# yhlleo/DWC-GAN

Hardware: AMD Instinct MI355X
Metric: CelebA 128x128 training images/sec (higher is better)
Workload: dtype f32; 1 GPU; BASELINE configs[1]: CelebA-shaped 128x128, per-GPU batch 16, fp32, full iteration (dis_update + gen_update + EMA + LR step), vgg_w=0, stride-1 3x3 / 5x5 and stride-2 4x4 layers (forward, data and weight gradient) as fp32-accurate TWO-plane f16 split products on the f16 MFMA (hi + lo 2^-11 per operand, per-tensor power-of-two scales, 3 products per multiply-add, matrix-core partial sums flushed to; image_size=128, per_gpu_batch=16, global_batch=16, parallelism=dp1

## Files before the change

### dwc-gan_amd/csrc/conv_halo_x3.hip

```cpp
#include <type_traits>

#include "conv_geom.h"

namespace {

typedef __bf16 bf16;
typedef __bf16 bf16x8 __attribute__((ext_vector_type(8)));
typedef unsigned int u32x2 __attribute__((ext_vector_type(2)));

constexpr int TB = 16;
constexpr int CS = 16;

typedef float f32x2 __attribute__((ext_vector_type(2)));
__device__ __forceinline__ void split3(f32x4 v, u32x2& p0, u32x2& p1, u32x2& p2) {
#pragma unroll
    for (int k = 0; k < 2; ++k) {
        const f32x2 x = {v[2 * k], v[2 * k + 1]};
        const f32x2 hb = {__uint_as_float(__float_as_uint(x[0]) & 0xffff0000u), __uint_as_float(__float_as_uint(x[1]) & 0xffff0000u)};
        const f32x2 r = x - hb;
        const f32x2 mb = {__uint_as_float(__float_as_uint(r[0]) & 0xffff0000u), __uint_as_float(__float_as_uint(r[1]) & 0xffff0000u)};
        const f32x2 l = r - mb;
        p0[k] = __builtin_amdgcn_perm(__float_as_uint(x[1]), __float_as_uint(x[0]), 0x07060302u);
        p1[k] = __builtin_amdgcn_perm(__float_as_uint(r[1]), __float_as_uint(r[0]), 0x07060302u);
        p2[k] = __builtin_amdgcn_perm(__float_as_uint(l[1]), __float_as_uint(l[0]), 0x07060302u);
// ... 32 lines not shown
    const bf16* w;
    const float* bias;
    const float* add;
    float* y;
    int B, H, W, Cin, N, rows, act, reflect;
    int blocks_x, blocks_per_img, tiles_n;
    float* part = nullptr;
    unsigned* tickets = nullptr;
    unsigned* status = nullptr;
    int split_from = 0;
    const unsigned long long* xs = nullptr;
    unsigned xs_epoch = 0;
    size_t w_elems = 0;
    unsigned long long* ys = nullptr;
    unsigned ys_epoch = 0;
};

template <int KS, int BN, int WM, int WN, int TM, int TN, int DBG = 0, int PB = 2, int S2 = 0, int KSP = 1, int NPL = 3, int RING = 0,
          bool ZP = false>
__global__ __launch_bounds__(64 * WM * WN, WM * WN == 4 ? 2 : 1) void conv_halo_x3_kernel(X3Args a) {
    static_assert(!ZP || S2 == 1, "ZP is the stride-2 forward's zero rule (the other forms take X3Args::reflect)");
#if defined(__HIP_DEVICE_COMPILE__)
    constexpr int NW = WM * WN, THREADS = 64 * NW;
    constexpr int PPT = THREADS / 4;
    static_assert((NW == 8 || NW == 4) && WM * TM * 32 == 256 && WN * TN * 32 == BN, "tile shape");
    static_assert(!S2 || KS == 2, "stride-2 form: 2x2 taps per parity");
    static_assert(KSP == 1 || (KSP == 2 && S2 != 2 && NW == 4 && TM * TN <= 4), "contraction split: the two-per-CU tile only");
    static_assert(!RING || (NPL == 2 && PB == 1 && ((S2 == 0 && (KS == 3 || KS == 5)) || S2 == 2)), "fused border ring: two-plane data gradients");
    constexpr int PW = TB + KS - 1;
    constexpr int NALT = RING ? (S2 == 2 ? 1 : ((KS - 1) / 2) * ((KS - 1) / 2 + 1) / 2) : 0;
    constexpr int PWA = PW + NALT;
    constexpr int PPIX = PW * PW;
    constexpr int PPASS = (PPIX + PPT - 1) / PPT;
    constexpr int PITCH = PWA * CS + 8;
    constexpr int P_PLANE = PWA * PITCH;
    constexpr int W_CHUNKS = NPL * BN * 2;
// ... 574 lines not shown
                    }
                    if constexpr (NPL == 2) v = v * sx.inv * sw.inv;
                    v += bv[n][q4];
#pragma unroll
                    for (int k = 0; k < 4; ++k) {
                        if constexpr (decltype(general)::value) v[k] = dwc_act_apply(v[k], a.act, col + k);
                        else v[k] = dwc_act_simple(v[k], slope);
                    }
                    if (a.add) v += adv[n][q4];
                    if constexpr (NPL == 2) y_am = max(max(y_am, max(dwc_abs_bits(v[0]), dwc_abs_bits(v[1]))), max(dwc_abs_bits(v[2]), dwc_abs_bits(v[3])));
                    if (!(DBG & 256)) *reinterpret_cast<f32x4*>(dst + col) = v;
                    else asm volatile("" ::"v"(v));
                }
        }
    };
    if (dwc_act_is_simple(a.act)) store(std::false_type{});
    else store(std::true_type{});
    if constexpr (NPL == 2) {
        __shared__ unsigned s_am[NW];
        dwc_amax_block_publish(a.ys, a.ys_epoch, y_am, s_am);
    }
#endif
}

__global__ void x3_weight_prepare_kernel(const float* __restrict__ w, bf16* __restrict__ out, int Cout, int Cin, int K, int rows,
                                         int kdim, int dgrad) {
    const int ncs = (kdim + CS - 1) / CS;
    const size_t total = (size_t)K * K * ncs * rows * CS;
    const size_t idx = (size_t)blockIdx.x * blockDim.x + threadIdx.x;
    if (idx >= total) return;
    const int j = idx % CS;
    size_t r = idx / CS;
// ... 38 lines not shown
    const int cs = r % ncs, tap = r / ncs;
    const int kh = tap / K, kw = tap - kh * K;
    const int kc = cs * CS + j;
    float v = 0.f;
    if (!dgrad) {
        if (row < Cout && kc < Cin) v = w[(((size_t)row * Cin + kc) * K + kh) * K + kw];
    } else {
        if (row < Cin && kc < Cout) v = w[(((size_t)kc * Cin + row) * K + (K - 1 - kh)) * K + (K - 1 - kw)];
    }
    v *= sw.s;
    const _Float16 h = (_Float16)v;
    const _Float16 l = (_Float16)(v - (float)h);
    const size_t base = ((size_t)(tap * ncs + cs) * 2 * rows + row) * CS + (j ^ (((row >> 3) & 1) << 3));
    out[base] = __builtin_bit_cast(unsigned short, h);
    out[base + (size_t)rows * CS] = __builtin_bit_cast(unsigned short, l);
}

__global__ __launch_bounds__(256) void absmax_kernel(const float* __restrict__ x, size_t n, unsigned long long* slot, unsigned epoch) {
    const size_t n4 = n >> 2;
    unsigned m = 0;
    const f32x4* x4 = reinterpret_cast<const f32x4*>(x);
    const size_t stride = (size_t)gridDim.x * 256;
    size_t i = (size_t)blockIdx.x * 256 + threadIdx.x;
    for (; i + 3 * stride < n4; i += 4 * stride) {
        const f32x4 a = x4[i], b = x4[i + stride], c = x4[i + 2 * stride], d = x4[i + 3 * stride];
#pragma unroll
        for (int k = 0; k < 4; ++k) m = max(max(m, dwc_abs_bits(a[k])), max(dwc_abs_bits(b[k]), max(dwc_abs_bits(c[k]), dwc_abs_bits(d[k]))));
    }
    for (; i < n4; i += stride) {
        const f32x4 a = x4[i];
// ... 312 lines not shown
    for (int c = 1; c <= smax && c * roles <= 2 * cus; ++c) {
        const int wgs = c * roles, rounds = (wgs + cus - 1) / cus;
        const double fill = (double)wgs / (rounds * cus) / (rounds > 1 ? 1.05 : 1.0);
        if (fill > best + 1e-9) best = fill, s = c;
    }
    *ups = (units + s - 1) / s;
    *splits = (units + *ups - 1) / *ups;
}

bool x3_ok(int B, int H, int W, int Cin, int N, int K) {
    return B > 0 && (K == 3 || K == 5) && H >= TB && W >= TB && !(H % TB) && !(W % TB) && Cin >= CS && !(Cin % CS) && N >= 32 &&
           !(N % 4);
}

template <int KS, int BN, int WM, int WN, int TM, int TN, int DBG = 0, int PB = 2, int S2 = 0, int KSP = 1, int NPL = 3, int RING = 0,
          bool ZP = false>
void x3_launch(const X3Args& a, dim3 grid, hipStream_t st) {
    hipLaunchKernelGGL((conv_halo_x3_kernel<KS, BN, WM, WN, TM, TN, DBG, PB, S2, KSP, NPL, RING, ZP>), grid, dim3(64 * WM * WN), 0, st, a);
}
size_t h2_w_elems(int rows, int kdim, int K) { return (size_t)K * K * ((kdim + CS - 1) / CS) * 2 * rows * CS; }

constexpr int X3_KSPLIT_TILES = 256, X3_KSPLIT_TICKETS = 512;
constexpr size_t X3_KSPLIT_TILE_BYTES = 256 * 64 * sizeof(float);
long x3_ksplit_from(long tiles, int slabs) {
    static const int on = getenv("DWC_X3_KSPLIT") ? atoi(getenv("DWC_X3_KSPLIT")) : 1;
    if (!on || slabs < 8 || (slabs & 1) || (tiles & 7)) return -1;
    return tiles <= X3_KSPLIT_TILES ? 0 : -1;
}
bool x3_ksplit_on(long tiles, int slabs) { return x3_ksplit_from(tiles, slabs) >= 0; }
size_t x3_ksplit_bytes(long tiles, int slabs) {
    const long from = x3_ksplit_from(tiles, slabs);
    return from < 0 ? 0 : (size_t)(tiles - from) * X3_KSPLIT_TILE_BYTES;
}
// ... 268 lines not shown

int dwc_x3_conv2d_s2_bwd_data(const float* dy, const void* w_prepared, float* dx, int B, int H, int W, int Cin, int Cout, int rows,
                              void* stream) {
    return x3_s2_bwd_data_impl<3>(dy, nullptr, 0, w_prepared, dx, B, H, W, Cin, Cout, rows, stream);
}
int dwc_h2_conv2d_s2_bwd_data(const float* dy, const void* dy_amax, unsigned dy_epoch, const void* w_prepared, float* dx, int B, int H, int W,
                              int Cin, int Cout, int rows, void* stream) {
    return x3_s2_bwd_data_impl<2>(dy, dy_amax, dy_epoch, w_prepared, dx, B, H, W, Cin, Cout, rows, stream);
}

int dwc_h2_conv2d_s2_bwd_data_fused(const float* dy, const void* dy_amax, unsigned dy_epoch, const void* w_prepared, float* dx, int B, int H,
                                    int W, int Cin, int Cout, int rows, void* stream) {
    return x3_s2_bwd_data_impl<2>(dy, dy_amax, dy_epoch, w_prepared, dx, B, H, W, Cin, Cout, rows, stream, true);
}

size_t dwc_x3_conv2d_wgrad_ws_bytes(int B, int H, int W, int Cin, int Cout, int K) {
    const int bn = x3_wgrad_bn(B, H, W, Cin, Cout, K);
    if (!bn) return 0;
    int splits = 0;
    for (int npl = 2; npl <= 3; ++npl) {
        int s, ups;
        x3_wgrad_plan(B, H, W, Cin, Cout, K, bn, npl, &s, &ups);
        splits = s > splits ? s : splits;
    }
    return (size_t)splits * (bn == 128 ? 1 : 2) * K * K * Cin * Cout * sizeof(float);
}

}

template <int NPL, bool ZP = false>
// ... 63 lines not shown
```

### dwc-gan_amd/hipdwc/_lib.py

```python
import ctypes
import os

_HERE = os.path.dirname(os.path.abspath(__file__))
LIB_PATH = os.environ.get("DWC_HIP_LIB") or os.path.join(os.path.dirname(_HERE), "lib", "libdwcgan_hip.so")

c_fp = ctypes.c_void_p
c_int = ctypes.c_int
c_sz = ctypes.c_size_t
c_f = ctypes.c_float
c_u = ctypes.c_uint


class AdvSpec(ctypes.Structure):
    _fields_ = [("target", c_f * 4), ("w_src", c_f * 4), ("w_cls", c_f * 4)]


BN_MAX_SEGMENTS = 8


TXT_MAX_LAYERS = 4


class TxtLayers(ctypes.Structure):
    _fields_ = [("n", c_int), ("out", c_fp * TXT_MAX_LAYERS), ("c", c_fp * TXT_MAX_LAYERS)]
# ... 129 lines not shown
    "dwc_x3_conv2d_wgrad_ws_bytes": (c_sz, [c_int] * 6),
    "dwc_x3_conv2d_wgrad": (c_int, [c_fp, c_fp, c_fp] + [c_int] * 8 + [c_fp, c_sz, c_fp]),
    "dwc_absmax": (c_int, [c_fp, c_sz, c_fp, c_u, c_fp]),
    "dwc_instnorm_fwd_amax": (c_int, [c_fp] * 7 + [c_int, c_int, c_int, c_f, c_int, c_fp, c_sz, c_fp, c_u, c_fp]),
    "dwc_instnorm_bwd_amax": (c_int, [c_fp] * 9 + [c_int, c_int, c_int, c_int, c_fp, c_sz, c_fp, c_u, c_fp]),
    "dwc_layernorm_fwd_amax": (c_int, [c_fp] * 6 + [c_int, c_int, c_int, c_f, c_int, c_fp, c_sz, c_fp, c_u, c_fp]),
    "dwc_layernorm_bwd_amax": (c_int, [c_fp] * 9 + [c_int, c_int, c_int, c_f, c_int, c_fp, c_sz, c_fp, c_u, c_fp]),
    "dwc_act_bwd_bias_amax": (c_int, [c_fp, c_fp, c_fp, c_fp, c_int, c_int, c_int, c_fp, c_sz, c_fp, c_u, c_fp]),
    "dwc_h2_weight_prepared_elems": (c_sz, [c_int] * 3),
    "dwc_h2_weight_prepare": (c_int, [c_fp, c_fp] + [c_int] * 5 + [c_fp, c_u, c_fp]),
    "dwc_h2_conv2d_same_add_ws": (c_int, [c_fp, c_fp, c_u] + [c_fp] * 4 + [c_fp, c_u] + [c_int] * 9 + [c_fp, c_sz, c_fp, c_fp]),
    "dwc_h2_conv2d_bwd_data_same_fused": (c_int, [c_fp, c_fp, c_u] + [c_fp] * 3 + [c_int] * 7 + [c_fp, c_sz, c_fp, c_fp]),
    "dwc_h2_conv2d_s2_ws": (c_int, [c_fp, c_fp, c_u] + [c_fp] * 3 + [c_fp, c_u] + [c_int] * 7 + [c_fp, c_sz, c_fp, c_fp]),
    "dwc_h2_conv2d_s2_bwd_data": (c_int, [c_fp, c_fp, c_u, c_fp, c_fp] + [c_int] * 6 + [c_fp]),
    "dwc_h2_conv2d_s2_bwd_data_fused": (c_int, [c_fp, c_fp, c_u, c_fp, c_fp] + [c_int] * 6 + [c_fp]),
    "dwc_h2_conv2d_wgrad": (c_int, [c_fp, c_fp, c_u, c_fp, c_fp, c_u, c_fp] + [c_int] * 8 + [c_fp, c_sz, c_fp]),
    "dwc_bf16_conv2d_wgrad_halo_ws_bytes": (c_sz, [c_int] * 6),
    "dwc_bf16_conv2d_wgrad_halo": (c_int, [c_fp, c_fp, c_fp] + [c_int] * 8 + [c_fp, c_sz, c_fp]),
    "dwc_bf16_conv7_smallk_wgrad_ws_bytes": (c_sz, [c_int] * 4),
    "dwc_bf16_conv7_smallk_wgrad": (c_int, [c_fp, c_fp, c_fp] + [c_int] * 5 + [c_fp, c_sz, c_fp]),
    "dwc_x3_conv7_smallk_wgrad_ws_bytes": (c_sz, [c_int] * 4),
    "dwc_x3_conv7_smallk_wgrad": (c_int, [c_fp, c_fp, c_fp] + [c_int] * 5 + [c_fp, c_sz, c_fp]),
    "dwc_bf16_conv2d_stem_ok": (c_int, [c_int] * 7),
    "dwc_bf16_conv2d_stem": (c_int, [c_fp] * 4 + [c_int] * 9 + [c_fp]),
    "dwc_bf16_conv2d_stem_crop": (c_int, [c_fp] * 5 + [c_int] * 10 + [c_fp]),
    "dwc_bf16_conv2d_narrow_ok": (c_int, [c_int] * 8),
    "dwc_bf16_conv2d_narrow": (c_int, [c_fp] * 4 + [c_int] * 12 + [c_fp]),
    "dwc_bf16_conv2d_bwd_data_image_narrow": (c_int, [c_fp, c_fp, c_fp] + [c_int] * 7 + [c_fp, c_sz, c_fp]),
    "dwc_bf16_conv2d_bwd_data_image_ws_bytes": (c_sz, [c_int] * 7),
    "dwc_bf16_conv2d_bwd_data_image": (c_int, [c_fp, c_fp, c_fp] + [c_int] * 7 + [c_fp, c_sz, c_fp]),
# ... 135 lines not shown
```

### dwc-gan_amd/hipdwc/ops.py

```python
import os
import weakref

import numpy as np
import torch

from . import _lib, derived

ACT = {"none": 0, None: 0, "relu": 1, "lrelu": 2, "tanh": 3, "sigmoid": 4, "heads": 5, "heads8": 6}

PRECISION = "fp32"
BF16 = torch.bfloat16

_REMOVED_SWITCHES = ("DWC_WINOGRAD", "DWC_TXT_STREAM", "DWC_NORM_FUSED_FINAL", "DWC_GEMM_TILE", "DWC_STRIP_BM", "DWC_X3_DUO", "DWC_X3_BN",
                     "DWC_X3_BN32", "DWC_X3_WIDE", "DWC_X3_STAGGER", "DWC_HALO_STAGGER", "DWC_X3_WDUO", "DWC_HALO16", "DWC_HALO_DUO",
                     "DWC_HALO_BN128", "DWC_BF16_TILE", "DWC_BF16_STAGES3", "DWC_NARROW_ROWS16")
_set = [k for k in _REMOVED_SWITCHES if k in os.environ]
if _set:
    import warnings
    warnings.warn("hipdwc: %s no longer select%s anything (removed in round 5, DESIGN.md 10.3) and %s ignored" % (
        ", ".join(_set), "s" if len(_set) == 1 else "", "is" if len(_set) == 1 else "are"), stacklevel=2)
del _set


def set_precision(name):
# ... 545 lines not shown

class ResGradToken:
    __slots__ = ("g",)

    def __init__(self):
        self.g = None


RES_FUSE = int(os.environ.get("DWC_RES_FUSE", "1"))


def res_token(x):
    return ResGradToken() if RES_FUSE and torch.is_grad_enabled() and x.requires_grad else None


_X3_TICKETS = {}


def _x3_ksplit(lib, dev, B, H, W, Cx, cop, K, stride, at_least=0):
    need = lib.dwc_x3_conv2d_ksplit_ws_bytes(B, H, W, Cx, cop, K, stride)
    if not need:
        ws = workspace(at_least, dev) if at_least else None
        return ws, at_least, None
    key = (_dev_index(dev), _stream())
    row = _X3_TICKETS.get(key)
    if row is None:
        row = torch.zeros(int(lib.dwc_x3_conv2d_ksplit_ticket_words()), dtype=torch.int32, device=dev)
        _X3_TICKETS[key] = row
    n = max(int(need), int(at_least))
    return workspace(n, dev), n, row.data_ptr()
# ... 148 lines not shown
    if x.dtype == BF16:
        ws = workspace(lib.dwc_bf16_conv7_smallk_wgrad_ws_bytes(B, H, W, int(swapped)), x.device)
        _lib.check(_timed("conv_wgrad_kernel+reduce", flops, lambda: lib.dwc_bf16_conv7_smallk_wgrad(
            a.data_ptr(), bt.data_ptr(), dw.data_ptr(), B, H, W, planes, int(swapped), ws.data_ptr(), ws.numel(), st),
            scope_name=scope_name, detail=kind + shape), "conv7_smallk_wgrad")
    else:
        ws = workspace(lib.dwc_x3_conv7_smallk_wgrad_ws_bytes(B, H, W, int(swapped)), x.device)
        _lib.check(_timed("wgrad_x3_kernel+reduce", flops, lambda: lib.dwc_x3_conv7_smallk_wgrad(
            a.data_ptr(), bt.data_ptr(), dw.data_ptr(), B, H, W, planes, int(swapped), ws.data_ptr(), ws.numel(), st),
            scope_name=scope_name, detail=kind + "-x3" + shape, exec_flops=6 * flops), "x3_conv7_smallk_wgrad")


class _Conv2d(torch.autograd.Function):

    @staticmethod
    def forward(ctx, x, w, b, stride, pad, act, bias_grad=True, owner=None, token=None, nograd=False, zero=False):
        _require_device(x)
        lib = _lib.load()
        x = cl(x)
        half = x.dtype == BF16
        ctx.token = token
        B, Cx, H, W = x.shape
        Cout, Cin, KH, KW = w.shape
        if Cin > Cx:
            raise ValueError("input has %d channels, weight expects %d" % (Cx, Cin))
        ctx.bias_grad = bias_grad
        ctx.zero_flag = bool(b is not None and getattr(b, "_dwc_zero_grad", False))
        ctx.owner = owner
        zero = bool(zero and pad > 0)
        ctx.zero = zero
        refl = 0 if zero else 1
        z = "_zeropad" if zero else ""
        cop = _padc(Cout, x.dtype)
# ... 47 lines not shown
                x.data_ptr(), w_hwio.data_ptr(), _p(bias), y.data_ptr(), B, H, W, Cx, cop, act, st),
                detail="fwd-s2halo" + shape), "conv2d_s2_halo")
        elif half and HALO and stride == 1 and KH == KW and 2 * pad == KH - 1 and lib.dwc_bf16_conv2d_same_halo_ok(B, H, W, Cx, cop, KH):
            _halo_same_bf16(lib, x, w, owner, "fwd", bias, None, y, B, H, W, Cx, cop, KH, act, refl, flops, "fwd-halo" + shape)
        else:
            w_hwio = _prepped(w, "fwd", cop, Cx, stride, owner, half)
            nws = _fn(lib, "conv2d_fwd_ws_bytes", x)(B, H, W, Cx, cop, KH, KW, stride, pad)
            wsp = _splitk_ws(nws, x.device)
            _lib.check(_timed("conv_gemm_kernel", flops, lambda: _fn(lib, "conv2d_fwd_zeropad" if zero else "conv2d_fwd", x)(
                x.data_ptr(), w_hwio.data_ptr(), _p(bias), y.data_ptr(), B, H, W, Cx, cop, KH, KW, stride, pad, act, wsp, nws,
                st), detail="fwd" + shape), "conv2d_fwd")
        ctx.save_for_backward(x, w, y if act != 0 else None)
        ctx.x_amax = getattr(x, "_dwc_amax", None)
        ctx.geom = (B, H, W, Cx, cop, KH, KW, stride, pad, act, Cin, Cout, b is not None)
        ctx.bscope = ("bwd:" + SCOPE) if SCOPE else ""
        return y

    @staticmethod
    def backward(ctx, dy):
        lib = _lib.load()
        x, w, y = ctx.saved_tensors
        B, H, W, Cx, cop, KH, KW, stride, pad, act, Cin, Cout, has_b = ctx.geom
        dy = cl(dy)
        Ho, Wo = dy.shape[2], dy.shape[3]
        need_db = has_b and ctx.needs_input_grad[2]
        g = dy
        db = None
        if need_db and not ctx.bias_grad:
            db, need_db = (None if ctx.zero_flag else torch.zeros(Cout, dtype=torch.float32, device=x.device)), False
        if act != 0 or need_db:
            g, db_full = _act_bwd(lib, dy, y, B, cop, Ho, Wo, act, need_db, slot=True)
            _hbm("act_bwd_bias", dy.numel() * dy.element_size() * ((1 if y is None else 2) + (1 if act != 0 else 0)))
            if need_db:
                db = db_full[:Cout]
        g_res = None
        if ctx.token is not None:
            g_res, ctx.token.g = ctx.token.g, None
            if g_res is not None:
                g_res = cl(g_res)
                if g_res.shape[1] != Cx or g_res.dtype != x.dtype or not ctx.needs_input_grad[0]:
                    raise RuntimeError("residual-gradient token: shape / dtype of the identity branch does not match the block input")
        flops = 2.0 * B * Ho * Wo * Cout * Cin * KH * KW
        shape = " B%d %dx%d %d>%d k%d s%d" % (B, H, W, Cx, cop, KH, stride)
        dx = dw = None
        if ctx.needs_input_grad[1]:
            dw = _Conv2d._wgrad(ctx, lib, x, g, w, flops, shape)
        if ctx.needs_input_grad[0]:
            same = stride == 1 and pad > 0 and 2 * pad == KH - 1 and KH == KW and cop >= 32 and (cop & (cop - 1)) == 0
            dx, used = (_Conv2d._dgrad_zero if ctx.zero else _Conv2d._dgrad_reflect)(ctx, lib, g, g_res, w, same, flops, shape)
            if used:
                g_res = None
        if g_res is not None and dx is not None:
            dx = dx + g_res.to(dx.dtype)
        return dx, dw, db, None, None, None, None, None, None, None, None

    @staticmethod
    def _wgrad(ctx, lib, x, g, w, flops, shape):
        B, H, W, Cx, cop, KH, KW, stride, pad, act, Cin, Cout, has_b = ctx.geom
        half = x.dtype == BF16
        dev, st = x.device, _stream()
        zero = ctx.zero
        dw = torch.empty((Cout, Cin, KH, KW), dtype=torch.float32, device=dev)
        z = "_zeropad" if zero else ""
        if (not zero) and Cout == 64 and (_stem_bf16(half, Cx, cop, KH, KW, stride, pad)
                                          or (SMALLK_X3 and _stem_x3(half, Cx, cop, KH, KW, stride, pad))):
            _smallk_wgrad(lib, x, g, dw, B, H, W, Cin, False, flops, ctx.bscope, "wgrad-stem", shape)
        elif ((not half) and (_x3_use(lib, B, H, W, Cx, cop, KH, KW, stride, pad)
                              or (X3 and X3_S2 and stride == 2 and KH == 4 and KW == 4 and pad == 1))
              and (KH != 3 or X3_WGRAD_HALO3) and (not zero or B * H * W * Cx * 4 < (1 << 31))
# ... 86 lines not shown
                _lib.check(_timed("conv_gemm_kernel", flops, lambda: _fn(lib, "conv2d_bwd_data_same", g)(
                    g.data_ptr(), w_dg(), w_dg_t(), dx.data_ptr(), B, H, W, Cx, cop, KH, KW, pad, ws.data_ptr(),
                    ws.numel(), st), scope_name=ctx.bscope, detail="dgrad" + shape), "conv2d_bwd_data_same")
                return dx, False
            _lib.check(_timed("conv_gemm_kernel" if half else "conv_halo_x3_kernel", 0.0, lambda: _fn(lib, "conv2d_bwd_data_ring", g)(
                g.data_ptr(), w_dg(), w_dg_t(), dx.data_ptr(), B, H, W, Cx, cop, KH, KW, pad, ws.data_ptr(), nws, st),
                scope_name=ctx.bscope, detail="dgrad-ring" + shape), "conv2d_bwd_data_ring")
            return dx, True
        if _s2_dgrad_halo_ok(lib, half, B, H, W, Cx, cop, KH, KW, stride, pad):
            fused = bool(RING_FUSED and (half or h2_fits(g)))
            w_dg = _prepped(w, "dgrad", cop, Cx, 2, owner, half) if half or not fused else None
            if half and fused:
                _lib.check(_timed("conv_gemm_kernel", flops, lambda: lib.dwc_bf16_conv2d_s2_halo_bwd_data_fused(
                    g.data_ptr(), w_dg.data_ptr(), dx.data_ptr(), B, H, W, Cx, cop, st), scope_name=ctx.bscope,
                    detail="dgrad-s2halo" + shape), "conv2d_s2_halo_bwd_data_fused")
            elif fused:
                w_h2 = _prepped(w, "h2_dgrad", cop, Cx, 1, owner)
                ga = amax_of(g)
                _lib.check(_timed("conv_halo_x3_kernel", flops, lambda: lib.dwc_h2_conv2d_s2_bwd_data_fused(
                    g.data_ptr(), ga[0], ga[1], w_h2.data_ptr(), dx.data_ptr(), B, H, W, Cx, cop, Cx, st), scope_name=ctx.bscope,
                    exec_flops=3 * flops, detail="dgrad-h2s2" + shape), "h2_conv2d_s2_bwd_data_fused")
            else:
                dxp = workspace(B * (H + 2) * (W + 2) * Cx * (2 if half else 4), dev)
                _s2_dgrad_halo(lib, g, w, owner, dx, B, H, W, Cx, cop, flops, ctx.bscope, shape)
                _lib.check(_timed("conv_gemm_kernel" if half else "conv_halo_x3_kernel", 0.0, lambda: _fn(lib, "conv2d_bwd_data_s2_ring", g)(
                    g.data_ptr(), w_dg.data_ptr(), dxp.data_ptr(), dx.data_ptr(), B, H, W, Cx, cop, st), scope_name=ctx.bscope,
                    detail="dgrad-ring" + shape), "conv2d_bwd_data_s2_ring")
            return dx, False
        _im2col_dgrad_reflect(lib, g, w, owner, dx, B, H, W, Cx, cop, KH, KW, stride, pad, flops, ctx.bscope, "dgrad" + shape)
        return dx, False

    @staticmethod
# ... 1 lines not shown
        B, H, W, Cx, cop, KH, KW, stride, pad, act, Cin, Cout, has_b = ctx.geom
        owner = ctx.owner
        dt = g.dtype
        half = dt == BF16
        dev = g.device
        dx = empty_cl(B, Cx, H, W, dev, dt)
        if same and (not half) and _x3_use(lib, B, H, W, cop, Cx, KH, KW, stride, pad, free=True):
            _sp_same(lib, g, w, owner, "dgrad", None, g_res, dx, B, H, W, Cx, cop, KH, 0, 0, flops, shape + " zeropad", " zeropad dgrad",
                     scope_name=ctx.bscope)
            return dx, True
        if same and half and HALO and lib.dwc_bf16_conv2d_same_halo_ok(B, H, W, cop, Cx, KH):
            _halo_same_bf16(lib, g, w, owner, "dgrad", None, g_res, dx, B, H, W, Cx, cop, KH, 0, 0, flops, "dgrad-halo" + shape + " zeropad",
                            " zeropad dgrad", ctx.bscope)
            return dx, True
        if _s2_dgrad_halo_ok(lib, half, B, H, W, Cx, cop, KH, KW, stride, pad):
            _s2_dgrad_halo(lib, g, w, owner, dx, B, H, W, Cx, cop, flops, ctx.bscope, shape + " zeropad", " zeropad")
            return dx, False
        w_dg = _prepped(w, "dgrad", cop, Cx, stride, owner, half)
        nws = _fn(lib, "conv2d_bwd_data_crop_ws_bytes", g)(B, H, W, Cx, cop, KH, KW, stride, pad)
        wsp = _splitk_ws(nws, dev)
        st = _stream()
        _lib.check(_timed("conv_gemm_kernel", flops, lambda: _fn(lib, "conv2d_bwd_data_crop", g)(
            g.data_ptr(), w_dg.data_ptr(), dx.data_ptr(), B, H, W, Cx, cop, KH, KW, stride, pad, wsp, nws, st),
            scope_name=ctx.bscope, detail="dgrad" + shape + " zeropad"), "conv2d_bwd_data_crop")
        return dx, False


_PAD_MODES = ("reflect", "zero")


def _pad_mode_zero(pad_mode):
    if pad_mode not in _PAD_MODES:
        raise ValueError("pad_mode %r: the HIP convolutions take %s" % (pad_mode, " / ".join(_PAD_MODES)))
    return pad_mode == "zero"


def conv2d(x, w, b, stride, pad, act="none", bias_grad=True, owner=None, token=None, pad_mode="reflect"):
    zero = _pad_mode_zero(pad_mode)
    if not bias_grad and ZERO_GRAD_BY_FLAG and isinstance(b, torch.nn.Parameter):
        b._dwc_zero_grad = True
    y = _Conv2d.apply(x, w, b, int(stride), int(pad), ACT[act], bool(bias_grad), owner, token, not torch.is_grad_enabled(), zero)
    return y if y.shape[1] == w.shape[0] else y[:, :w.shape[0]]


def conv2d_padded(x, w, b, stride, pad, act="none", pad_mode="reflect"):
    return _Conv2d.apply(x, w, b, int(stride), int(pad), ACT[act], True, None, None, False, _pad_mode_zero(pad_mode))


class _HeadsConvWide(torch.autograd.Function):

    @staticmethod
    def forward(ctx, x, w4, b4, owner=None):
        _require_device(x)
        lib = _lib.load()
        x = cl(x)
        half = x.dtype == BF16
# ... 900 lines not shown
```

### dwc-gan_amd/networks/networks.py

```python
import torch
import torch.nn.functional as F
from torch import nn

from hipdwc import batchnorm, ops, spectral

_CONV_ACTS = ("relu", "lrelu", "tanh", "sigmoid", "none")
_NORM_ACTS = ("relu", "lrelu", "none")


class AdaptiveInstanceNorm2d(nn.Module):

    def __init__(self, num_features, eps=1e-5, momentum=0.1):
        super().__init__()
        self.num_features, self.eps, self.momentum = num_features, eps, momentum
        self.weight = None
        self.bias = None
        self.register_buffer("running_mean", torch.zeros(num_features))
        self.register_buffer("running_var", torch.ones(num_features))

    def forward(self, x, relu=False, residual=None, token=None, act=None):
        if self.weight is None or self.bias is None:
            raise AssertionError("Please assign weight and bias before calling AdaIN!")
        return ops.instance_norm(x, self.weight, self.bias, residual=residual, relu=relu, eps=self.eps, token=token, act=act)

# ... 90 lines not shown
        else:
            raise AssertionError("Unsupported normalization: {}".format(norm))
        if activation == "prelu":
            self.activation = nn.PReLU()
        self.conv = nn.Conv2d(input_dim, output_dim, kernel_size, stride, bias=self.use_bias)
        if norm == "sn":
            self.conv = SpectralNorm(self.conv)

    def _torch_act(self, y):
        if self.act_kind == "prelu":
            return self.activation(y)
        if self.act_kind == "selu":
            return torch.nn.functional.selu(y)
        return {"lrelu": lambda t: torch.nn.functional.leaky_relu(t, 0.1), "tanh": torch.tanh, "sigmoid": torch.sigmoid}[self.act_kind](y)

    def forward(self, x, residual=None, conv_token=None, res_token=None, sn=None, segments=None, stat_order=None):
        if x.shape[1] < 4:
            x = ops.pack_image(x)
        pad = self.padding
        mode = "zero" if self.pad_type == "zero" and ops.ZERO_PAD_HIP else "reflect"
        if self.pad_type != "reflect" and mode != "zero" and pad > 0:
            if self.stride != 1:
                raise NotImplementedError("pad_type=%r with stride %d needs hipdwc.ops.ZERO_PAD_HIP = 1" % (self.pad_type, self.stride))
            x = torch.nn.functional.pad(x, (pad,) * 4, mode="constant" if self.pad_type == "zero" else "replicate")
            pad = 0
        fused_act = self.act_kind in _CONV_ACTS
        if self.norm_kind == "sn":
            if sn is None:
                sn = spectral.sn_power_iteration([self.conv.module], segments or 1)
            y = spectral.sn_conv2d(x, self.conv.module, sn, self.stride, pad, self.act_kind if fused_act else "none", token=conv_token,
                                   pad_mode=mode)
            if not fused_act:
                y = self._torch_act(y)
            return y if residual is None else y + residual
        if self.norm is None:
            y = ops.conv2d(x, self.conv.weight, self.conv.bias, self.stride, pad, self.act_kind if fused_act else "none", token=conv_token,
                           pad_mode=mode)
            if not fused_act:
                y = self._torch_act(y)
            return y if residual is None else y + residual
        if self.norm_kind == "bn":
            bias = self.conv.bias
            train = self.norm.training or not self.norm.track_running_stats
            if not train and getattr(bias, "_dwc_zero_grad", False):
                bias._dwc_zero_grad = False
            y = ops.conv2d(x, self.conv.weight, bias, self.stride, pad, "none", bias_grad=not train, token=conv_token, pad_mode=mode)
            fused = self.act_kind in batchnorm.ACTS
            y = self.norm(y, act=self.act_kind if fused else "none", segments=segments, stat_order=stat_order)
            if not fused:
                y = self._torch_act(y)
            return y if residual is None else y + residual
        if self.act_kind not in (_NORM_ACTS if ops.NORM_ACT_FUSED else ("relu", "none")):
            y = ops.conv2d(x, self.conv.weight, self.conv.bias, self.stride, pad, "none", token=conv_token, pad_mode=mode)
            y = self.norm(y) if self.norm_kind == "ln" else self.norm(y, relu=False)
            y = torch.relu(y) if self.act_kind == "relu" else (y if self.act_kind == "none" else self._torch_act(y))
            return y if residual is None else y + residual
        y = ops.conv2d(x, self.conv.weight, self.conv.bias, self.stride, pad, "none",
                       bias_grad=self.norm_kind == "ln", token=conv_token,
                       pad_mode=mode)
        if self.norm_kind == "ln":
            y = self.norm(y, act=self.act_kind)
            return y if residual is None else y + residual
        return self.norm(y, act=self.act_kind, residual=residual, token=res_token)


class ResBlock(nn.Module):

    def __init__(self, dim, norm="in", activation="relu", pad_type="zero"):
        super().__init__()
        self.model = nn.Sequential(
            Conv2dBlock(dim, dim, 3, 1, 1, norm=norm, activation=activation, pad_type=pad_type),
            Conv2dBlock(dim, dim, 3, 1, 1, norm=norm, activation="none", pad_type=pad_type))

    def forward(self, x, groups=1):
        fused = self.model[1].norm_kind in ("in", "adain")
        if groups > 1:
            return self._forward_groups(x, groups)
        token = ops.res_token(x) if fused else None
# ... 161 lines not shown
    def bn_layers(self, num_scales=None):
        n = self.num_scales if num_scales is None else num_scales
        return [blk.norm for s in range(n) for blk in self.cnns_feat[s] if blk.norm_kind == "bn"]

    def forward(self, x, use_multiscales=True, segments=None, stat_order=None):
        x = ops.pack_image(x)
        outputs = []
        layers = self.sn_layers(self.num_scales if use_multiscales else 1)
        sn = spectral.sn_power_iteration(layers, segments or 1) if layers else None
        for s in range(self.num_scales):
            if self.norm == "bn":
                h = x
                for blk in self.cnns_feat[s]:
                    h = blk(h, segments=segments, stat_order=stat_order) if blk.norm_kind == "bn" else blk(h)
            elif sn is None:
                h = self.cnns_feat[s](x)
            else:
                h = x
                for blk in self.cnns_feat[s]:
                    h = blk(h, sn=sn)
            src = ops.conv2d(h, self.cnns_src[s].weight, self.cnns_src[s].bias, 1, 0).float()
            cls = ops.conv2d(h, self.cnns_cls[s].weight, None, 1, 0).float()
            outputs.append([src, cls.reshape(cls.size(0), -1)])
            if not use_multiscales:
                break
            if s + 1 < self.num_scales:
                x = ops.downsample_half(x)
        return outputs

    def forward_src_scale0_torch(self, x):
        if self.norm not in ("none", "sn", "in", "ln") or self.pad_type not in ("reflect", "zero", "replicate"):
# ... 128 lines not shown
```

### dwc-gan_amd/networks/networks_v2.py

```python
import numpy as np
import torch
from torch import nn

from hipdwc import host, ops, txt
from .networks import ContentEncoder, MLP, Conv2dBlock, ResBlocks, AdaptiveInstanceNorm2d, Decoder


class HeadList(list):
    flat = None

    @classmethod
    def of(cls, flat, k):
        out = cls(flat.reshape(flat.shape[0], k, -1).unbind(1))
        out.flat = flat
        return out

    def rows(self, a, b):
        return HeadList.of(self.flat[a:b], len(self))


def flat_heads(heads):
    if torch.is_tensor(heads):
        return heads
    flat = getattr(heads, "flat", None)
# ... 11 lines not shown
            convs.append(Conv2dBlock(dim, nxt, 4, 2, 1, norm=norm, activation=activ, pad_type=pad_type))
            dim = nxt
        convs.append(nn.AdaptiveAvgPool2d(1))
        self.model = nn.Sequential(*convs)
        if use_map:
            self.mapping = nn.Sequential(nn.Linear(dim, dim), nn.ReLU(inplace=True), nn.Dropout(p=0.1),
                                         nn.Linear(dim, dim), nn.ReLU(inplace=True))
        self.fcs, self.fcvars = nn.ModuleList(), nn.ModuleList()
        for _ in range(num_class):
            self.fcs.append(nn.Linear(dim, c_dim))
            self.fcvars.append(nn.Linear(dim, c_dim))
        self.output_dim = dim

    def forward(self, x, drop_mask=None):
        h = ops.pack_image(x) if x.shape[1] < 4 else x
        for blk in list(self.model)[:-1]:
            h = blk(h)
        f = h.float().mean(dim=(2, 3))
        if self.use_map:
            f = ops.linear(f, self.mapping[0].weight, self.mapping[0].bias, "relu")
            if self.training and self.mapping[2].p > 0:
                if drop_mask is None:
                    drop_mask = host.noise().dropout_mask(f.shape, self.mapping[2].p, f.device)
                f = f * drop_mask
            f = ops.linear(f, self.mapping[3].weight, self.mapping[3].bias, "relu")
        heads_w = [m.weight for m in self.fcs] + [m.weight for m in self.fcvars]
        w = ops.cat_params(heads_w)
        b = ops.cat_params([m.bias for m in self.fcs] + [m.bias for m in self.fcvars])
        out = ops.linear(f, w, b, owner=tuple(heads_w))
        k, c = self.num_class, self.c_dim
        return HeadList.of(out[:, :k * c], k), HeadList.of(out[:, k * c:2 * k * c], k)

# ... 199 lines not shown
```

### include/dwcgan_hip.h

```cpp
#ifndef DWCGAN_HIP_H
#define DWCGAN_HIP_H

#include <stddef.h>
#include <stdint.h>

#ifdef __cplusplus
extern "C" {
#endif

#define DWC_OK 0
#define DWC_EINVAL (-1)
#define DWC_EWORKSPACE (-2)
#define DWC_ELAUNCH (-3)

#define DWC_ACT_NONE 0
#define DWC_ACT_RELU 1
#define DWC_ACT_LRELU 2
#define DWC_ACT_TANH 3
#define DWC_ACT_SIGMOID 4
#define DWC_ACT_HEADS 5
#define DWC_ACT_HEADS8 6

#define DWC_ABI_VERSION 11
int dwc_version(void);
// ... 239 lines not shown
int dwc_h2_weight_prepare(const float* w_oihw, void* out, int Cout, int Cin, int K, int rows, int dgrad, const void* w_amax,
                          unsigned w_epoch, void* stream);
int dwc_h2_conv2d_same_add_ws(const float* x, const void* x_amax, unsigned x_epoch, const void* w_prepared, const float* bias,
                              const float* add, float* y, void* y_amax, unsigned y_epoch, int B, int H, int W, int Cin, int N, int rows,
                              int K, int act, int reflect, void* ws, size_t ws_bytes, unsigned* tickets, void* stream);
int dwc_h2_conv2d_bwd_data_same_fused(const float* dy, const void* dy_amax, unsigned dy_epoch, const void* w_prepared, const float* add,
                                      float* dx, int B, int H, int W, int Cout, int N, int rows, int K, void* ws, size_t ws_bytes,
                                      unsigned* tickets, void* stream);
int dwc_h2_conv2d_s2_ws(const float* x, const void* x_amax, unsigned x_epoch, const void* w_prepared, const float* bias, float* y,
                        void* y_amax, unsigned y_epoch, int B, int H, int W, int Cin, int N, int rows, int act, void* ws, size_t ws_bytes,
                        unsigned* tickets, void* stream);
int dwc_h2_conv2d_s2_bwd_data(const float* dy, const void* dy_amax, unsigned dy_epoch, const void* w_prepared, float* dx, int B, int H, int W,
                              int Cin, int Cout, int rows, void* stream);
int dwc_h2_conv2d_s2_bwd_data_fused(const float* dy, const void* dy_amax, unsigned dy_epoch, const void* w_prepared, float* dx, int B, int H,
                                    int W, int Cin, int Cout, int rows, void* stream);
int dwc_h2_conv2d_wgrad(const float* x, const void* x_amax, unsigned x_epoch, const float* dy, const void* dy_amax, unsigned dy_epoch,
                        float* dw_oihw, int B, int H, int W, int Cin, int Cout, int K, int cin_real, int cout_real, void* ws, size_t ws_bytes,
                        void* stream);
size_t dwc_x3_conv2d_wgrad_ws_bytes(int B, int H, int W, int Cin, int Cout, int K);
int dwc_x3_conv2d_wgrad(const float* x, const float* dy, float* dw_oihw, int B, int H, int W, int Cin, int Cout, int K, int cin_real,
                        int cout_real, void* ws, size_t ws_bytes, void* stream);

size_t dwc_bf16_weight_prepared_elems(int Cout, int Cin, int KH, int KW, int stride, int cout_pad, int cin_pad, int for_dgrad);
int dwc_bf16_weight_prepare_fwd(const float* w_oihw, void* w_prepared, int Cout, int Cin, int KH, int KW, int cout_pad,
                                int cin_pad, void* stream);
int dwc_bf16_weight_prepare_dgrad(const float* w_oihw, void* w_prepared, int Cout, int Cin, int KH, int KW, int stride,
                                  int cout_pad, int cin_pad, void* stream);
size_t dwc_bf16_conv2d_fwd_ws_bytes(int B, int H, int W, int Cin, int Cout, int KH, int KW, int stride, int pad);
int dwc_bf16_conv2d_fwd(const void* x, const void* w_prepared, const float* bias, void* y, int B, int H, int W, int Cin,
                        int Cout, int KH, int KW, int stride, int pad, int act, void* ws, size_t ws_bytes, void* stream);
// ... 237 lines not shown
```

Baseline: 402.7 images/s.

## Fuse previous layer's activation backward and bias-gradient sum into stride-2 data gradient

After: 403.2 images/s, median of 2. About the same (+0.1%).

```diff
diff --git a/dwc-gan_amd/csrc/conv_halo_x3.hip b/dwc-gan_amd/csrc/conv_halo_x3.hip
--- a/dwc-gan_amd/csrc/conv_halo_x3.hip
+++ b/dwc-gan_amd/csrc/conv_halo_x3.hip
@@ -70,12 +70,18 @@
     size_t w_elems = 0;
     unsigned long long* ys = nullptr;
     unsigned ys_epoch = 0;
+    const float* gate_y = nullptr;
+    int gate_act = 0;
+    float gate_slope = 0.1f;
+    float* db_part = nullptr;
 };
 
 template <int KS, int BN, int WM, int WN, int TM, int TN, int DBG = 0, int PB = 2, int S2 = 0, int KSP = 1, int NPL = 3, int RING = 0,
-          bool ZP = false>
+          bool ZP = false, bool GATE = false>
 __global__ __launch_bounds__(64 * WM * WN, WM * WN == 4 ? 2 : 1) void conv_halo_x3_kernel(X3Args a) {
     static_assert(!ZP || S2 == 1, "ZP is the stride-2 forward's zero rule (the other forms take X3Args::reflect)");
+    static_assert(!GATE || (S2 == 2 && NPL == 2 && KSP == 1 && WN == 1 && TN == 2 && DBG == 0),
+                  "GATE: the two-plane stride-2 data gradient (every stored pixel final, 64 columns per wave)");
 #if defined(__HIP_DEVICE_COMPILE__)
     constexpr int NW = WM * WN, THREADS = 64 * NW;
     constexpr int PPT = THREADS / 4;
@@ -680,8 +686,80 @@
                 }
         }
     };
-    if (dwc_act_is_simple(a.act)) store(std::false_type{});
-    else store(std::true_type{});
+    if constexpr (GATE) {
+        const bool gated = a.gate_act != DWC_ACT_NONE, sums = a.db_part != nullptr;
+        const float gslope = a.gate_act == DWC_ACT_RELU ? 0.f : a.gate_slope;
+        constexpr int NC = TN * 16;
+        float csum[NC];
+#pragma unroll
+        for (int j = 0; j < NC; ++j) csum[j] = 0.f;
+#pragma unroll
+        for (int i = 0; i < TM; ++i) {
+            const int pb = (wm * TM + i) * 32 + l31;
+            const size_t e0 = ((size_t)(n_img * 2 * OH + 2 * (y0 + (pb >> 4)) + ry) * (2 * OW) + 2 * (x0 + (pb & 15)) + rx) * a.N;
+#pragma unroll
+            for (int n = 0; n < TN; ++n) {
+                f32x4 adv[4], gyv[4];
+#pragma unroll
+                for (int q4 = 0; q4 < 4; ++q4) adv[q4] = f32x4{0.f, 0.f, 0.f, 0.f}, gyv[q4] = f32x4{1.f, 1.f, 1.f, 1.f};
+                if (a.add) {
+#pragma unroll
+                    for (int q4 = 0; q4 < 4; ++q4)
+                        adv[q4] = *reinterpret_cast<const f32x4*>(a.add + e0 + min(n0 + n * 32 + 8 * q4 + 4 * hi, a.N - 4));
+                }
+                if (gated) {
+#pragma unroll
+                    for (int q4 = 0; q4 < 4; ++q4)
+                        gyv[q4] = *reinterpret_cast<const f32x4*>(a.gate_y + e0 + min(n0 + n * 32 + 8 * q4 + 4 * hi, a.N - 4));
+                }
+#pragma unroll
+                for (int q4 = 0; q4 < 4; ++q4) {
+                    const int col = n0 + n * 32 + 8 * q4 + 4 * hi;
+                    const bool ok = col < a.N;
+                    f32x4 v = {acc[i][n][4 * q4], acc[i][n][4 * q4 + 1], acc[i][n][4 * q4 + 2], acc[i][n][4 * q4 + 3]};
+                    v = v * sx.inv * sw.inv;
+                    v += f32x4{0.f, 0.f, 0.f, 0.f};
+                    v += adv[q4];
+                    {
+#pragma clang fp contract(off)
+#pragma unroll
+                        for (int k = 0; k < 4; ++k) {
+                            v[k] = v[k] * (gyv[q4][k] > 0.f ? 1.f : gslope);
+                            csum[(n * 4 + q4) * 4 + k] += ok ? v[k] : 0.f;
+                        }
+                    }
+                    if (ok) {
+                        y_am = max(max(y_am, max(dwc_abs_bits(v[0]), dwc_abs_bits(v[1]))), max(dwc_abs_bits(v[2]), dwc_abs_bits(v[3])));
+                        *reinterpret_cast<f32x4*>(a.y + e0 + col) = v;
+                    }
+                }
+            }
+        }
+        if (sums) {
+            static_assert(NC == 32, "reduce-scatter over 32 lanes");
+#pragma unroll
+            for (int o = 16; o >= 1; o >>= 1) {
+                const bool up = (l31 & o) != 0;
+#pragma unroll
+                for (int j = 0; j < o; ++j) {
+                    const float keep = up ? csum[j + o] : csum[j], send = up ? csum[j] : csum[j + o];
+                    csum[j] = keep + __shfl_xor(send, o, 64);
+                }
+            }
+            __shared__ float s_db[NW][64];
+            s_db[wave][(l31 >> 4) * 32 + ((l31 >> 2) & 3) * 8 + 4 * hi + (l31 & 3)] = csum[0];
+            __syncthreads();
+            if (t < 64 && n0 + t < a.N) {
+                float s = s_db[0][t];
+#pragma unroll
+                for (int w = 1; w < NW; ++w) s += s_db[w][t];
+                a.db_part[((size_t)blk * 4 + 2 * ry + rx) * a.N + n0 + t] = s;
+            }
+        }
+    } else {
+        if (dwc_act_is_simple(a.act)) store(std::false_type{});
+        else store(std::true_type{});
+    }
     if constexpr (NPL == 2) {
         __shared__ unsigned s_am[NW];
         dwc_amax_block_publish(a.ys, a.ys_epoch, y_am, s_am);
@@ -750,6 +828,31 @@
     const size_t base = ((size_t)(tap * ncs + cs) * 2 * rows + row) * CS + (j ^ (((row >> 3) & 1) << 3));
     out[base] = __builtin_bit_cast(unsigned short, h);
     out[base + (size_t)rows * CS] = __builtin_bit_cast(unsigned short, l);
+}
+
+__global__ __launch_bounds__(1024) void gate_colsum_final(const float* __restrict__ part, float* __restrict__ out, int rows, int C) {
+    __shared__ float sm[16][64];
+    const int cl = threadIdx.x & 63, g = threadIdx.x >> 6;
+    const int c = blockIdx.x * 64 + cl;
+    float s = 0.f;
+    if (c < C) {
+        int k = g;
+        for (; k + 7 * 16 < rows; k += 8 * 16) {
+            float v[8];
+#pragma unroll
+            for (int u = 0; u < 8; ++u) v[u] = part[(size_t)(k + 16 * u) * C + c];
+#pragma unroll
+            for (int u = 0; u < 8; ++u) s += v[u];
+        }
+        for (; k < rows; k += 16) s += part[(size_t)k * C + c];
+    }
+    sm[g][cl] = s;
+    __syncthreads();
+    if (g == 0 && c < C) {
+#pragma unroll
+        for (int k = 1; k < 16; ++k) s += sm[k][cl];
+        out[c] = s;
+    }
 }
 
 __global__ __launch_bounds__(256) void absmax_kernel(const float* __restrict__ x, size_t n, unsigned long long* slot, unsigned epoch) {
@@ -1092,9 +1195,9 @@
 }
 
 template <int KS, int BN, int WM, int WN, int TM, int TN, int DBG = 0, int PB = 2, int S2 = 0, int KSP = 1, int NPL = 3, int RING = 0,
-          bool ZP = false>
+          bool ZP = false, bool GATE = false>
 void x3_launch(const X3Args& a, dim3 grid, hipStream_t st) {
-    hipLaunchKernelGGL((conv_halo_x3_kernel<KS, BN, WM, WN, TM, TN, DBG, PB, S2, KSP, NPL, RING, ZP>), grid, dim3(64 * WM * WN), 0, st, a);
+    hipLaunchKernelGGL((conv_halo_x3_kernel<KS, BN, WM, WN, TM, TN, DBG, PB, S2, KSP, NPL, RING, ZP, GATE>), grid, dim3(64 * WM * WN), 0, st, a);
 }
 size_t h2_w_elems(int rows, int kdim, int K) { return (size_t)K * K * ((kdim + CS - 1) / CS) * 2 * rows * CS; }
 
@@ -1393,6 +1496,37 @@
     return x3_s2_bwd_data_impl<2>(dy, dy_amax, dy_epoch, w_prepared, dx, B, H, W, Cin, Cout, rows, stream, true);
 }
 
+size_t dwc_h2_conv2d_s2_bwd_data_gated_ws_bytes(int B, int H, int W, int Cin) {
+    if (B <= 0 || H < 2 * TB || W < 2 * TB || Cin <= 0) return 0;
+    return (size_t)B * (H / (2 * TB)) * (W / (2 * TB)) * 4 * Cin * sizeof(float);
+}
+int dwc_h2_conv2d_s2_bwd_data_gated(const float* dy, const void* dy_amax, unsigned dy_epoch, const void* w_prepared, const float* add,
+                                    float* dx, int B, int H, int W, int Cin, int Cout, int rows, int ring, const float* y, int act,
+                                    float slope, float* db_full, void* ws, size_t ws_bytes, void* g_amax, unsigned g_epoch, void* stream) {
+    if (!dy || !w_prepared || !dx || !dy_amax || !x3_s2_ok(B, H, W, Cout, Cin) || (size_t)B * H * W * Cin >= 0x7fffffffull || rows < Cin ||
+        (size_t)B * (H / 2) * (W / 2) * Cout * 4 >= 0x80000000ull || act < DWC_ACT_NONE || act > DWC_ACT_LRELU || (act != DWC_ACT_NONE && !y))
+        return DWC_EINVAL;
+    if (db_full && (!ws || ws_bytes < dwc_h2_conv2d_s2_bwd_data_gated_ws_bytes(B, H, W, Cin))) return DWC_EWORKSPACE;
+    X3Args a;
+    a.x = dy; a.w = (const bf16*)w_prepared; a.bias = nullptr; a.add = add; a.y = dx;
+    a.xs = (const unsigned long long*)dy_amax; a.xs_epoch = dy_epoch; a.w_elems = h2_w_elems(rows, Cout, 4);
+    a.ys = (unsigned long long*)g_amax; a.ys_epoch = g_epoch;
+    a.B = B; a.H = H / 2; a.W = W / 2; a.Cin = Cout; a.N = Cin; a.rows = rows; a.act = DWC_ACT_NONE; a.reflect = 0;
+    a.blocks_x = (W / 2) / TB; a.blocks_per_img = ((H / 2) / TB) * ((W / 2) / TB);
+    a.tiles_n = (Cin + 63) / 64;
+    a.gate_y = y; a.gate_act = act; a.gate_slope = slope; a.db_part = db_full ? (float*)ws : nullptr;
+    const int tiles = B * a.blocks_per_img;
+    const dim3 grid(4 * tiles * a.tiles_n);
+    if (ring) x3_launch<2, 64, 4, 1, 2, 2, 0, 1, 2, 1, 2, 1, false, true>(a, grid, (hipStream_t)stream);
+    else x3_launch<2, 64, 4, 1, 2, 2, 0, 1, 2, 1, 2, 0, false, true>(a, grid, (hipStream_t)stream);
+    DWC_LAUNCH_CHECK();
+    if (db_full) {
+        hipLaunchKernelGGL(gate_colsum_final, dim3((Cin + 63) / 64), dim3(1024), 0, (hipStream_t)stream, (const float*)ws, db_full, 4 * tiles, Cin);
+        DWC_LAUNCH_CHECK();
+    }
+    return DWC_OK;
+}
+
 size_t dwc_x3_conv2d_wgrad_ws_bytes(int B, int H, int W, int Cin, int Cout, int K) {
     const int bn = x3_wgrad_bn(B, H, W, Cin, Cout, K);
     if (!bn) return 0;
diff --git a/dwc-gan_amd/hipdwc/_lib.py b/dwc-gan_amd/hipdwc/_lib.py
--- a/dwc-gan_amd/hipdwc/_lib.py
+++ b/dwc-gan_amd/hipdwc/_lib.py
@@ -167,6 +167,9 @@
     "dwc_h2_conv2d_s2_ws": (c_int, [c_fp, c_fp, c_u] + [c_fp] * 3 + [c_fp, c_u] + [c_int] * 7 + [c_fp, c_sz, c_fp, c_fp]),
     "dwc_h2_conv2d_s2_bwd_data": (c_int, [c_fp, c_fp, c_u, c_fp, c_fp] + [c_int] * 6 + [c_fp]),
     "dwc_h2_conv2d_s2_bwd_data_fused": (c_int, [c_fp, c_fp, c_u, c_fp, c_fp] + [c_int] * 6 + [c_fp]),
+    "dwc_h2_conv2d_s2_bwd_data_gated_ws_bytes": (c_sz, [c_int] * 4),
+    "dwc_h2_conv2d_s2_bwd_data_gated": (c_int, [c_fp, c_fp, c_u, c_fp, c_fp, c_fp] + [c_int] * 7 + [c_fp, c_int, c_f, c_fp, c_fp, c_sz, c_fp,
+                                                                                                  c_u, c_fp]),
     "dwc_h2_conv2d_wgrad": (c_int, [c_fp, c_fp, c_u, c_fp, c_fp, c_u, c_fp] + [c_int] * 8 + [c_fp, c_sz, c_fp]),
     "dwc_bf16_conv2d_wgrad_halo_ws_bytes": (c_sz, [c_int] * 6),
     "dwc_bf16_conv2d_wgrad_halo": (c_int, [c_fp, c_fp, c_fp] + [c_int] * 8 + [c_fp, c_sz, c_fp]),
diff --git a/dwc-gan_amd/hipdwc/ops.py b/dwc-gan_amd/hipdwc/ops.py
--- a/dwc-gan_amd/hipdwc/ops.py
+++ b/dwc-gan_amd/hipdwc/ops.py
@@ -583,6 +583,24 @@
     return ResGradToken() if RES_FUSE and torch.is_grad_enabled() and x.requires_grad else None
 
 
+class GateToken:
+    __slots__ = ("y", "act", "need_db", "g", "db_full")
+
+    def __init__(self):
+        self.y = self.g = self.db_full = None
+        self.act, self.need_db = 0, False
+
+    def output(self):
+        return self.y() if self.y is not None else None
+
+
+GATE_FUSED = int(os.environ.get("DWC_GATE_FUSED", "1"))
+
+
+def gate_token():
+    return GateToken() if GATE_FUSED and torch.is_grad_enabled() else None
+
+
 _X3_TICKETS = {}
 
 
@@ -761,9 +779,13 @@
 class _Conv2d(torch.autograd.Function):
 
     @staticmethod
-    def forward(ctx, x, w, b, stride, pad, act, bias_grad=True, owner=None, token=None, nograd=False, zero=False):
+    def forward(ctx, x, w, b, stride, pad, act, bias_grad=True, owner=None, token=None, nograd=False, zero=False, gate=None):
         _require_device(x)
         lib = _lib.load()
+        gate_in, gate_out = gate if gate is not None else (None, None)
+        gy = gate_in.output() if gate_in is not None else None
+        ctx.gate_in = gate_in if (gy is not None and x.data_ptr() == gy.data_ptr() and x.shape == gy.shape and x.dtype == gy.dtype
+                                  and x.is_contiguous(memory_format=torch.channels_last)) else None
         x = cl(x)
         half = x.dtype == BF16
         ctx.token = token
@@ -841,6 +863,11 @@
         ctx.x_amax = getattr(x, "_dwc_amax", None)
         ctx.geom = (B, H, W, Cx, cop, KH, KW, stride, pad, act, Cin, Cout, b is not None)
         ctx.bscope = ("bwd:" + SCOPE) if SCOPE else ""
+        ctx.gate_out = None
+        if gate_out is not None and not half and act <= ACT["lrelu"] and Cout == cop:
+            gate_out.y, gate_out.act = weakref.ref(y), act
+            gate_out.need_db = bool(b is not None and ctx.needs_input_grad[2] and bias_grad and not nograd)
+            ctx.gate_out = gate_out
         return y
 
     @staticmethod
@@ -853,9 +880,21 @@
         need_db = has_b and ctx.needs_input_grad[2]
         g = dy
         db = None
+        gated = False
+        if ctx.gate_out is not None and ctx.gate_out.g is not None:
+            tok = ctx.gate_out
+            g, db_full, tok.g, tok.db_full = tok.g, tok.db_full, None, None
+            if dy.data_ptr() != g.data_ptr() or dy.shape != g.shape:
+                raise RuntimeError("gate token: the gradient of this convolution's output is not the tensor its declared only consumer "
+                                   "wrote -- the output has a second consumer, which GateToken's caller must rule out")
+            gated = True
+            if need_db and ctx.bias_grad:
+                if db_full is None:
+                    _, db_full = _act_bwd(lib, g, None, B, cop, Ho, Wo, 0, True)
+                db, need_db = db_full[:Cout], False
         if need_db and not ctx.bias_grad:
             db, need_db = (None if ctx.zero_flag else torch.zeros(Cout, dtype=torch.float32, device=x.device)), False
-        if act != 0 or need_db:
+        if (act != 0 or need_db) and not gated:
             g, db_full = _act_bwd(lib, dy, y, B, cop, Ho, Wo, act, need_db, slot=True)
             _hbm("act_bwd_bias", dy.numel() * dy.element_size() * ((1 if y is None else 2) + (1 if act != 0 else 0)))
             if need_db:
@@ -879,7 +918,31 @@
                 g_res = None
         if g_res is not None and dx is not None:
             dx = dx + g_res.to(dx.dtype)
-        return dx, dw, db, None, None, None, None, None, None, None, None
+        return dx, dw, db, None, None, None, None, None, None, None, None, None
+
+    @staticmethod
+    def _gated_s2_dgrad(ctx, lib, g, w, dx, ring, flops, shape):
+        B, H, W, Cx, cop, KH, KW, stride, pad, act, Cin, Cout, has_b = ctx.geom
+        tok = ctx.gate_in
+        w_h2 = _prepped(w, "h2_dgrad", cop, Cx, 1, ctx.owner)
+        ga = amax_of(g)
+        da, dep = out_amax(dx)
+        y = ctx.saved_tensors[0]
+        db_full = torch.empty(Cx, dtype=torch.float32, device=g.device) if tok.need_db else None
+        nws = lib.dwc_h2_conv2d_s2_bwd_data_gated_ws_bytes(B, H, W, Cx) if tok.need_db else 0
+        ws = torch.empty(nws, dtype=torch.uint8, device=g.device) if nws else None
+        st = _stream()
+        _lib.check(_timed("conv_halo_x3_kernel", flops, lambda: lib.dwc_h2_conv2d_s2_bwd_data_gated(
+            g.data_ptr(), ga[0], ga[1], w_h2.data_ptr(), None, dx.data_ptr(), B, H, W, Cx, cop, Cx, int(ring),
+            y.data_ptr() if tok.act != 0 else None, tok.act, 0.1, _p(db_full), _p(ws), nws, da, dep, st), scope_name=ctx.bscope,
+            exec_flops=3 * flops, detail="dgrad-h2s2" + shape), "h2_conv2d_s2_bwd_data_gated")
+        set_amax(dx, da, dep)
+        tok.g, tok.db_full = dx, db_full
+
+    @staticmethod
+    def _gate_ready(ctx, g, g_res):
+        return bool(GATE_FUSED and ctx.gate_in is not None and g_res is None and g.dtype == torch.float32 and h2_fits(g)
+                    and h2_fits(ctx.saved_tensors[0]))
 
     @staticmethod
     def _wgrad(ctx, lib, x, g, w, flops, shape):
@@ -996,8 +1059,10 @@
                 _lib.check(_timed("conv_gemm_kernel", flops, lambda: lib.dwc_bf16_conv2d_s2_halo_bwd_data_fused(
                     g.data_ptr(), w_dg.data_ptr(), dx.data_ptr(), B, H, W, Cx, cop, st), scope_name=ctx.bscope,
                     detail="dgrad-s2halo" + shape), "conv2d_s2_halo_bwd_data_fused")
+            elif fused and _Conv2d._gate_ready(ctx, g, g_res):
+                _Conv2d._gated_s2_dgrad(ctx, lib, g, w, dx, True, flops, shape)
             elif fused:
-                w_h2 = _prepped(w, "h2_dgrad", cop, Cx, 1, owner)
+                w_h2 =_prepped(w, "h2_dgrad", cop, Cx, 1, owner)
                 ga = amax_of(g)
                 _lib.check(_timed("conv_halo_x3_kernel", flops, lambda: lib.dwc_h2_conv2d_s2_bwd_data_fused(
                     g.data_ptr(), ga[0], ga[1], w_h2.data_ptr(), dx.data_ptr(), B, H, W, Cx, cop, Cx, st), scope_name=ctx.bscope,
@@ -1029,6 +1094,9 @@
                             " zeropad dgrad", ctx.bscope)
             return dx, True
         if _s2_dgrad_halo_ok(lib, half, B, H, W, Cx, cop, KH, KW, stride, pad):
+            if _Conv2d._gate_ready(ctx, g, g_res):
+                _Conv2d._gated_s2_dgrad(ctx, lib, g, w, dx, False, flops, shape + " zeropad")
+                return dx, False
             _s2_dgrad_halo(lib, g, w, owner, dx, B, H, W, Cx, cop, flops, ctx.bscope, shape + " zeropad", " zeropad")
             return dx, False
         w_dg = _prepped(w, "dgrad", cop, Cx, stride, owner, half)
@@ -1050,11 +1118,12 @@
     return pad_mode == "zero"
 
 
-def conv2d(x, w, b, stride, pad, act="none", bias_grad=True, owner=None, token=None, pad_mode="reflect"):
+def conv2d(x, w, b, stride, pad, act="none", bias_grad=True, owner=None, token=None, pad_mode="reflect", gate=None):
     zero = _pad_mode_zero(pad_mode)
     if not bias_grad and ZERO_GRAD_BY_FLAG and isinstance(b, torch.nn.Parameter):
         b._dwc_zero_grad = True
-    y = _Conv2d.apply(x, w, b, int(stride), int(pad), ACT[act], bool(bias_grad), owner, token, not torch.is_grad_enabled(), zero)
+    y = _Conv2d.apply(x, w, b, int(stride), int(pad), ACT[act], bool(bias_grad), owner, token, not torch.is_grad_enabled(), zero,
+                      gate if GATE_FUSED else None)
     return y if y.shape[1] == w.shape[0] else y[:, :w.shape[0]]
 
 
diff --git a/dwc-gan_amd/networks/networks.py b/dwc-gan_amd/networks/networks.py
--- a/dwc-gan_amd/networks/networks.py
+++ b/dwc-gan_amd/networks/networks.py
@@ -128,7 +128,8 @@
             return torch.nn.functional.selu(y)
         return {"lrelu": lambda t: torch.nn.functional.leaky_relu(t, 0.1), "tanh": torch.tanh, "sigmoid": torch.sigmoid}[self.act_kind](y)
 
-    def forward(self, x, residual=None, conv_token=None, res_token=None, sn=None, segments=None, stat_order=None):
+    def forward(self, x, residual=None, conv_token=None, res_token=None, sn=None, segments=None, stat_order=None, gate_in=None,
+                gate_out=None):
         if x.shape[1] < 4:
             x = ops.pack_image(x)
         pad = self.padding
@@ -149,7 +150,7 @@
             return y if residual is None else y + residual
         if self.norm is None:
             y = ops.conv2d(x, self.conv.weight, self.conv.bias, self.stride, pad, self.act_kind if fused_act else "none", token=conv_token,
-                           pad_mode=mode)
+                           pad_mode=mode, gate=(gate_in, gate_out if fused_act and residual is None else None))
             if not fused_act:
                 y = self._torch_act(y)
             return y if residual is None else y + residual
@@ -158,24 +159,36 @@
             train = self.norm.training or not self.norm.track_running_stats
             if not train and getattr(bias, "_dwc_zero_grad", False):
                 bias._dwc_zero_grad = False
-            y = ops.conv2d(x, self.conv.weight, bias, self.stride, pad, "none", bias_grad=not train, token=conv_token, pad_mode=mode)
+            y = ops.conv2d(x, self.conv.weight, bias, self.stride, pad, "none", bias_grad=not train, token=conv_token, pad_mode=mode,
+                           gate=(gate_in, None))
             fused = self.act_kind in batchnorm.ACTS
             y = self.norm(y, act=self.act_kind if fused else "none", segments=segments, stat_order=stat_order)
             if not fused:
                 y = self._torch_act(y)
             return y if residual is None else y + residual
         if self.act_kind not in (_NORM_ACTS if ops.NORM_ACT_FUSED else ("relu", "none")):
-            y = ops.conv2d(x, self.conv.weight, self.conv.bias, self.stride, pad, "none", token=conv_token, pad_mode=mode)
+            y = ops.conv2d(x, self.conv.weight, self.conv.bias, self.stride, pad, "none", token=conv_token, pad_mode=mode,
+                           gate=(gate_in, None))
             y = self.norm(y) if self.norm_kind == "ln" else self.norm(y, relu=False)
             y = torch.relu(y) if self.act_kind == "relu" else (y if self.act_kind == "none" else self._torch_act(y))
             return y if residual is None else y + residual
         y = ops.conv2d(x, self.conv.weight, self.conv.bias, self.stride, pad, "none",
                        bias_grad=self.norm_kind == "ln", token=conv_token,
-                       pad_mode=mode)
+                       pad_mode=mode, gate=(gate_in, None))
         if self.norm_kind == "ln":
             y = self.norm(y, act=self.act_kind)
             return y if residual is None else y + residual
         return self.norm(y, act=self.act_kind, residual=residual, token=res_token)
+
+
+def run_chain(blocks, h, **kw):
+    blocks = list(blocks)
+    tok = None
+    for i, blk in enumerate(blocks):
+        nxt = ops.gate_token() if i + 1 < len(blocks) else None
+        h = blk(h, gate_in=tok, gate_out=nxt, **kw)
+        tok = nxt
+    return h
 
 
 class ResBlock(nn.Module):
@@ -367,7 +380,7 @@
                 for blk in self.cnns_feat[s]:
                     h = blk(h, segments=segments, stat_order=stat_order) if blk.norm_kind == "bn" else blk(h)
             elif sn is None:
-                h = self.cnns_feat[s](x)
+                h = run_chain(self.cnns_feat[s], x)
             else:
                 h = x
                 for blk in self.cnns_feat[s]:
diff --git a/dwc-gan_amd/networks/networks_v2.py b/dwc-gan_amd/networks/networks_v2.py
--- a/dwc-gan_amd/networks/networks_v2.py
+++ b/dwc-gan_amd/networks/networks_v2.py
@@ -3,7 +3,7 @@
 from torch import nn
 
 from hipdwc import host, ops, txt
-from .networks import ContentEncoder, MLP, Conv2dBlock, ResBlocks, AdaptiveInstanceNorm2d, Decoder
+from .networks import ContentEncoder, MLP, Conv2dBlock, ResBlocks, AdaptiveInstanceNorm2d, Decoder, run_chain
 
 
 class HeadList(list):
@@ -49,8 +49,7 @@
 
     def forward(self, x, drop_mask=None):
         h = ops.pack_image(x) if x.shape[1] < 4 else x
-        for blk in list(self.model)[:-1]:
-            h = blk(h)
+        h = run_chain(list(self.model)[:-1], h)
         f = h.float().mean(dim=(2, 3))
         if self.use_map:
             f = ops.linear(f, self.mapping[0].weight, self.mapping[0].bias, "relu")
diff --git a/include/dwcgan_hip.h b/include/dwcgan_hip.h
--- a/include/dwcgan_hip.h
+++ b/include/dwcgan_hip.h
@@ -277,6 +277,10 @@
                               int Cin, int Cout, int rows, void* stream);
 int dwc_h2_conv2d_s2_bwd_data_fused(const float* dy, const void* dy_amax, unsigned dy_epoch, const void* w_prepared, float* dx, int B, int H,
                                     int W, int Cin, int Cout, int rows, void* stream);
+size_t dwc_h2_conv2d_s2_bwd_data_gated_ws_bytes(int B, int H, int W, int Cin);
+int dwc_h2_conv2d_s2_bwd_data_gated(const float* dy, const void* dy_amax, unsigned dy_epoch, const void* w_prepared, const float* add,
+                                    float* dx, int B, int H, int W, int Cin, int Cout, int rows, int ring, const float* y, int act,
+                                    float slope, float* db_full, void* ws, size_t ws_bytes, void* g_amax, unsigned g_epoch, void* stream);
 int dwc_h2_conv2d_wgrad(const float* x, const void* x_amax, unsigned x_epoch, const float* dy, const void* dy_amax, unsigned dy_epoch,
                         float* dw_oihw, int B, int H, int W, int Cin, int Cout, int K, int cin_real, int cout_real, void* ws, size_t ws_bytes,
                         void* stream);
```
